# dselivanov/rsparse

Hardware: AMD Instinct MI355X
Metric: als_iterations_per_sec (higher is better)
Workload: dtype f32 (Gram products of rows > 512 / <= 32 non-zeros as 2 x fp16 / 3 x bf16 split terms of the fp32 operands, fp32 accumulate; everything else fp32); 1 GPU; WRMF implicit ALS, CG(3), synthetic 10000000x1000000, 500155883 nnz, rank 128, lambda 0.1; survey_config=3, feedback=implicit, n_items=1000000, nnz=500155883, rank=128, solver=conjugate_gradient, cg_steps=3, parallelism=rows sharded x1, factors replicated

## Files before the change

rsparse_amd/build.py:

```python
import subprocess
import sys
import time
from concurrent.futures import ThreadPoolExecutor
from pathlib import Path

PKG = Path(__file__).resolve().parent
CSRC = PKG / "csrc"
SRC = [CSRC / n for n in ("wrmf_kernels.hip", "wrmf_cgq.hip", "wrmf_cgp.hip", "wrmf_ne.hip", "wrmf_chol.hip", "wrmf_chol_wave.hip", "wrmf_chol_mf.hip", "wrmf_cg_mf.hip", "wrmf_chol_lr.hip",
                          "wrmf_topk.hip", "wrmf_topk_large.hip", "wrmf_similar.hip", "wrmf_metrics.hip", "wrmf_hits.hip", "wrmf_lists.hip", "wrmf_diversity.hip", "wrmf_mmr.hip", "wrmf_ranks.hip", "wrmf_score.hip", "wrmf_softals.hip", "wrmf_itemknn.hip", "wrmf_candidates.hip", "wrmf_sample.hip", "wrmf_sample_weighted.hip", "wrmf_split.hip", "wrmf_confidence.hip", "wrmf_events.hip", "wrmf_explain.hip", "wrmf_init.hip", "wrmf_ingest.hip", "wrmf_nnls.hip", "wrmf_bias.hip", "wrmf_lu.hip",
                          "wrmf_f64.hip", "wrmf_wide.hip", "wrmf_wide_cg.hip", "wrmf_ctx_kernels.hip", "wrmf_schedule.cpp", "wrmf_capi.cpp", "wrmf_f64_capi.cpp", "wrmf_capi_host.cpp", "wrmf_ctx.cpp")]
HEADERS = [CSRC / "wrmf_chol_mf.attrs.csv", CSRC / "wrmf_mf.h", CSRC / "wrmf_internal.h", CSRC / "wrmf_capi_common.h", CSRC / "wrmf_schedule.h", CSRC / "wrmf_device.h", CSRC / "wrmf_sample_team.h", CSRC / "wrmf_wave.h", CSRC / "wrmf_csr_rows.h", CSRC / "wrmf_ldlt.h", CSRC / "wrmf_f64.h", CSRC / "wrmf_topk_plan.h", CSRC / "wrmf_ctx_layout.h", PKG.parent / "include" / "rsparse_wrmf_hip.h"]
DEPS = SRC + HEADERS
OUT = PKG / "lib" / "librsparse_wrmf_hip.so"
FLAGS = ["--offload-arch=gfx950", "-O3", "-std=c++17", "-fPIC"]


EXTRA_FLAGS = {n: ["-mllvm", "-forceattrs-csv-path=" + str(CSRC / "wrmf_chol_mf.attrs.csv"), "-fno-slp-vectorize"] for n in ("wrmf_chol_mf.hip", "wrmf_cg_mf.hip")}
AUDITED = {"wrmf_chol_mf.hip", "wrmf_cg_mf.hip"}
REG_LIMIT = {"wrmf_cg_mf.hip": 512}
NO_SPILL = {"wrmf_cgq.hip": ("14als_cgq_kernelILi128ELi24ELi4ELi4E",),
            "wrmf_cgp.hip": ("14als_cgp_kernelILb0ELb1ELi16ELb1E",),
            "wrmf_explain.hip": ("14explain_kernelIfLi128E",),
            "wrmf_sample.hip": ("13sample_kernelILi64E", "13sample_kernelILi256E"),
            "wrmf_sample_weighted.hip": ("22sample_weighted_kernelILi64E", "22sample_weighted_kernelILi256E"),
            "wrmf_hits.hip": ("18hit_metrics_kernelILb0E", "18hit_metrics_kernelILb1E"),
            "wrmf_lists.hip": ("19list_metrics_kernelILb0E", "19list_metrics_kernelILb1E"),
            "wrmf_diversity.hip": ("21list_diversity_kernelI", "21item_inv_norms_kernelI"),
            "wrmf_mmr.hip": ("10mmr_kernelI",),
            "wrmf_confidence.hip": ("conf_moments_kernel", "conf_moments_finish_kernel", "conf_table_kernel", "conf_apply_kernel"),
            "wrmf_events.hip": ("events_pack_kernel", "events_now_kernel", "events_heads_kernel", "events_reduce_kernel",
                                "events_long_chunks_kernel", "events_long_finish_kernel"),
            "wrmf_cg_mf.hip": ("rsparse_hip_als_cg_mf_implicit", "rsparse_hip_als_cg_mf_implicit_any"),
            "wrmf_softals.hip": ("softals_span_kernel", "softals_finish_kernel", "softals_empty_rows_kernel"),
            "wrmf_itemknn.hip": ("knn_scatter_kernel", "knn_mask_kernel", "knn_select_kernel", "knn_gather_kernel", "knn_cand_select_kernel",
                                 "knn_ranks_kernel"),
            "wrmf_split.hip": ("split_count_wave_kernel", "split_count_team_kernel", "split_write_wave_kernel", "split_write_team_kernel")}
RESOURCE_FLAG = "-Rpass-analysis=kernel-resource-usage"


def resource_violations(remarks, patterns, limit=256):
    import re
    rows, cur = [], None
    for line in remarks.splitlines():
        m = re.search(r"remark:\s+(.*?) \[-Rpass", line)
        if not m:
            continue
        t = m.group(1).strip()
        if t.startswith("Function Name:"):
            cur = {"name": t.split(":", 1)[1].strip()}
            rows.append(cur)
        elif ":" in t and cur is not None:
            k, v = t.rsplit(":", 1)
            cur[k.strip()] = v.strip()
# ... 94 lines not shown
```

rsparse_amd/csrc/wrmf_capi.cpp:

```cpp
#include "../../include/rsparse_wrmf_hip.h"

#include <cxxabi.h>

#include <algorithm>
#include <cfloat>
#include <cmath>
#include <cstdio>
#include <cstdlib>
#include <cstring>
#include <string>
#include <vector>

#include "wrmf_capi_common.h"
#include "wrmf_topk_plan.h"

using namespace rsparse_hip;

struct rsparse_hip_csc {
  DevCSC d;
  int device = 0;
  std::vector<void*> owned;
};

namespace {
// ... 114 lines not shown
  *out = static_cast<const T*>(p);
  return RSPARSE_HIP_OK;
}

int upload_cut(rsparse_hip_csc& m, const NeCut& cut, NeListSet& L) {
  L = NeListSet();
  L.entries = (int)cut.items.size();
  L.nseg = cut.nseg();
  L.nsplit = (int)cut.split_rows.size();
  if (int rc = upload(m, cut.segs, &L.segs)) return rc;
  if (int rc = upload(m, cut.split_rows, &L.split_rows)) return rc;
  return upload(m, cut.split_ptr, &L.split_ptr);
}
int upload_deal(rsparse_hip_csc& m, const NeDeal& deal, NeListSet& L) {
  L.wg = deal.wg();
  if (int rc = upload(m, deal.rows, &L.rows)) return rc;
  return upload(m, deal.ptr, &L.ptr);
}

int build_schedule(rsparse_hip_csc& m, const int32_t* host_col_ptrs) {
  DevCSC& d = m.d;
  int cus = 256;
  HIP_TRY(hipDeviceGetAttribute(&cus, hipDeviceAttributeMultiprocessorCount, m.device));
  d.q_cfg = cgq_default_cfg();
  SchedulePlan plan;
  if (!plan_schedule(host_col_ptrs, d.n_cols, cus, [](int len) { return cgq_bucket_of(len, cgq_default_cfg()); }, plan))
    return fail(RSPARSE_HIP_ERR_INVALID, "col_ptrs is not non-decreasing");
  d.max_len = plan.max_len; d.nnz_long = plan.nnz_long; d.n_empty = plan.n_empty;
  d.short_max = kTileNnz; d.n_long = plan.n_long;
  for (int b = 0; b < 7; b++) d.q_off[b] = plan.off[b];
  for (int b = 0; b < 6; b++) d.q_nnz[b] = plan.nnz[b];
  d.q_pair_first = plan.pair_first; d.q_team4_first = plan.team4_first;
  d.q_team4_wide_first = plan.team4_wide_first;
  d.q_gt32 = plan.gt32; d.q_gt48 = plan.gt48; d.q_lr_first = plan.lr_first; d.q_n_lr = plan.n_lr;
  d.q_n_chol_long = plan.n_chol_long; d.q_n_nec = plan.n_nec;
  int rc;
  if ((rc = upload(m, plan.order, &d.q_order))) return rc;
  if ((rc = upload(m, plan.stream_off, &d.q_stream_off))) return rc;
  if ((rc = upload_cut(m, plan.cut, d.q_ne))) return rc;
  d.q_ne1 = d.q_ne;
  if ((rc = upload_deal(m, plan.fine, d.q_ne))) return rc;
  if ((rc = upload_deal(m, plan.coarse, d.q_ne1))) return rc;
  if (plan.nec_is_ne) {
    d.q_nec = d.q_ne;
  } else {
    if ((rc = upload_cut(m, plan.cut_nec, d.q_nec))) return rc;
    if ((rc = upload_deal(m, plan.nec, d.q_nec))) return rc;
  }
  return RSPARSE_HIP_OK;
}

bool use_cgq(int rank, const void* X, const void* Y) {
  return rank % 4 == 0 && ((reinterpret_cast<uintptr_t>(X) | reinterpret_cast<uintptr_t>(Y)) & 15) == 0;
}

int check_common(int n_rows, int n_cols, const void* col_ptrs, const void* X, const void* Y, int rank) {
  if (n_rows < 0 || n_cols < 0) return fail(RSPARSE_HIP_ERR_INVALID, "negative matrix dimension");
  if (!col_ptrs) return fail(RSPARSE_HIP_ERR_INVALID, "col_ptrs is NULL");
  if (!X || !Y) return fail(RSPARSE_HIP_ERR_INVALID, "X or Y is NULL");
  if (rank <= 0) return fail(RSPARSE_HIP_ERR_INVALID, "rank must be positive");
  if (rank > RSPARSE_HIP_MAX_RANK)
    return fail(RSPARSE_HIP_ERR_UNSUPPORTED, "rank > 256 is not on the device path");
  return RSPARSE_HIP_OK;
}

thread_local int64_t g_fail_carry[2] = {0, 0};
// ... 84 lines not shown
    const int grid = wide_als_grid(d.n_cols);
    const int grid_w = wide_cg_wave_grid(d.n_cols) + wide_cg_team_grid(d.n_cols);
    if ((rc = g_ws.ensure_partials((size_t)grid + (size_t)grid_w))) return rc;
    HIP_TRY(g_ws.wide_m2.ensure(solver == RSPARSE_SOLVER_NNLS ? (size_t)grid * wide_m2_floats_per_wg(rank) : 0));
    HIP_TRY(g_ws.wide_lu.ensure(solver == RSPARSE_SOLVER_CHOLESKY ? (size_t)grid * rank * rank : 0));
    AlsArgs a{};
    a.col_ptrs = d.col_ptrs; a.row_idx = d.row_idx; a.vals = d.vals;
    a.X = d_X; a.Y = d_Y; a.XtX = implicit ? d_XtX : nullptr;
    a.n_cols = d.n_cols; a.k = rank; a.cg_steps = (int)cg_steps;
    a.lambda = (float)lambda; a.lambda_loss = lambda; a.dynamic_lambda = dynamic_lambda ? 1 : 0;
    a.loss_partials = g_ws.partials; a.fail_counter = g_ws.fails;
    a.rhs_vals = bias ? bias->rhs_vals : nullptr;
    a.loss_tgt = bias ? bias->loss_tgt : nullptr;
    a.rhs_init = bias ? bias->rhs_init : nullptr;
    a.loss_tgt_const = bias ? bias->tgt_const : 1.f;
    a.gbias = (solver == RSPARSE_SOLVER_CONJUGATE_GRADIENT && implicit && bias) ? bias->gbias : 0.f;
    const bool wave_cg = wide_cg_wave_supported(a, solver) && (d.q_order || d.max_len <= kWideCgMaxLen);
    hipError_t we = wave_cg ? launch_wide_cg_wave(a, implicit, kWideCgMaxLen, d.max_len > kWideCgMaxLen ? d.q_order : nullptr, 0, s)
                            : launch_als_wide(a, implicit, solver, g_ws.wide_m2, g_ws.wide_lu, s);
    if (we != hipSuccess) return hip_fail(we, wave_cg ? "launch_wide_cg_wave" : "launch_als_wide");
    if ((we = launch_sum_partials(g_ws.partials, wave_cg ? (size_t)grid_w : (size_t)grid, outw, s, g_ws.partials + g_ws.partial_slots())) != hipSuccess)
      return hip_fail(we, "launch_sum_partials");
    return RSPARSE_HIP_OK;
  }
  const bool cg = solver == RSPARSE_SOLVER_CONJUGATE_GRADIENT;
  const bool cgq = cg && use_cgq(rank, d_X, d_Y);
  QSchedule qs;
  qs.order = d.q_order;
  qs.cfg = d.q_cfg;
  qs.pair_first = d.q_pair_first;
  for (int b = 0; b < 7; b++) qs.off[b] = d.q_off[b];
  qs.team4_first = (implicit && bias && bias->gbias != 0.f) ? d.q_off[2] : d.q_team4_first;
  qs.team4_wide_first = (implicit && bias && bias->gbias != 0.f) ? d.q_off[2] : d.q_team4_wide_first;
  qs.pair_wide = cgp_wide_supported(rank, implicit, implicit && bias && bias->gbias != 0.f);
  qs.pair_quad = cgp_quad_supported(rank, implicit, implicit && bias && bias->gbias != 0.f);
  const bool cg_mf = cgq && implicit && !bias && cg_mf_supported(rank, implicit) && d.q_order && d.q_off[1] > d.q_n_nec;
  if (cg_mf) {
    qs.mf_rows = d.q_order + d.q_n_nec;
    qs.mf_n = d.q_off[1] - d.q_n_nec;
  }
  const bool chol_mf = chol_mf_supported(rank) && !cg && solver == RSPARSE_SOLVER_CHOLESKY && !bias && d.q_order && ne_supported(rank) &&
                       use_cgq(rank, d_X, d_Y) && d.q_lr_first > d.q_off[1];
  const int mf_first = d.q_off[1];
  const int n_mf = chol_mf ? d.q_lr_first - mf_first : 0;
  const bool nec_lists = padded_rank(rank) > 64 && d.q_nec.wg > 0 && !chol_mf;
  const bool ne_chol = !cg && solver == RSPARSE_SOLVER_CHOLESKY && !bias && (nec_lists || d.q_ne.wg > 0 || chol_mf) &&
                       ne_supported(rank) && use_cgq(rank, d_X, d_Y);
  qs.ne = (cg_mf || (ne_chol && nec_lists)) ? d.q_nec : ((implicit && padded_rank(rank) == 128) ? d.q_ne : d.q_ne1);
  const size_t chol_base = chol2_loss_slots(d.n_cols);
  const size_t slots = cgq ? cgq_loss_slots(qs, rank, implicit) : (cg ? cg_loss_slots(d.n_cols, d.n_long)
                                   : (solver == RSPARSE_SOLVER_NNLS ? chol_loss_slots(d.n_cols)
                                      : chol_base + (ne_chol ? (size_t)(qs.ne.entries + qs.ne.nsplit) : 0) +
                                            (size_t)(chol_mf ? chol_mf_loss_slots(n_mf, implicit) : 0) + (size_t)kLuGrid));
  if ((rc = g_ws.ensure_partials(slots))) return rc;
  double* out = d_loss_rows_out ? d_loss_rows_out : g_ws.scalars;
  if (d.n_cols == 0) {
    HIP_TRY(hipMemsetAsync(out, 0, sizeof(double), s));
    return RSPARSE_HIP_OK;
  }
  AlsArgs a;
  a.col_ptrs = d.col_ptrs; a.row_idx = d.row_idx; a.vals = d.vals;
  a.X = d_X; a.Y = d_Y; a.XtX = implicit ? d_XtX : nullptr;
  a.long_rows = d.n_long ? d.q_order : nullptr; a.n_long = d.n_long; a.n_cols = d.n_cols;
  a.chol_long_rows = d.q_order; a.n_chol_long = d.q_order ? d.q_n_chol_long : 0;
  a.chol_list = nullptr; a.chol_first = 0; a.chol_n_main = 0; a.chol_empty_first = 0;
  a.lr_rows = nullptr; a.n_lr = 0; a.lr_flags = nullptr; a.lr_M = nullptr; a.lr_n_gt32 = a.lr_n_gt16 = a.lr_n_gt48 = -1; a.lrx = 0;
// ... 1429 lines not shown
```

rsparse_amd/csrc/wrmf_cgq.hip:

```cpp
#include <algorithm>

#include "wrmf_internal.h"
#include "wrmf_device.h"

namespace rsparse_hip {
namespace {

using namespace dev;

constexpr int kGvFirstMinCapq = 16;
constexpr int kStreamPrefixQ = 4;
constexpr int kIdxPrefetchMaxWpr = 2;

constexpr int kMaxSavedSweeps = 4;

template <int KP>
struct QG {
  static constexpr int RPN = KP / 16;
  static constexpr int VW = RPN >= 4 ? 4 : RPN;
  static constexpr int NV = RPN / VW;
  __device__ static __forceinline__ int elem(int i, int r) { return (r / VW) * (16 * VW) + i * VW + (r % VW); }
};

template <int VW>
struct Piece;
template <>
struct Piece<4> { using type = float4; };
template <>
struct Piece<2> { using type = float2; };

__device__ __forceinline__ float groups_reduce_scatter4(const float a0, const float a1, const float a2, const float a3) {
  const auto s01 = __builtin_amdgcn_permlane16_swap(__float_as_uint(a0), __float_as_uint(a1), false, false);
  const float c = __uint_as_float(s01[0]) + __uint_as_float(s01[1]);
  const auto s23 = __builtin_amdgcn_permlane16_swap(__float_as_uint(a2), __float_as_uint(a3), false, false);
  const float d = __uint_as_float(s23[0]) + __uint_as_float(s23[1]);
  const auto t = __builtin_amdgcn_permlane32_swap(__float_as_uint(c), __float_as_uint(d), false, false);
  return __uint_as_float(t[0]) + __uint_as_float(t[1]);
}
template <int KP, int CAPQ, int WAVES, int WPR, int STREAM, bool IMPLICIT, int DMF = 0>
struct QSmem {
  static constexpr size_t gram_floats = (IMPLICIT && DMF != 1) ? (size_t)KP * KP : 0;
  static constexpr size_t vec_floats = IMPLICIT ? (size_t)WAVES * KP : 0;
  static constexpr size_t red_floats = WPR > 1 ? (size_t)2 * WAVES * KP + 2 * WAVES : 0;
  static constexpr bool cv_lds = !STREAM && CAPQ * (KP / 16) > 128;
  static constexpr bool wideq = !STREAM && CAPQ * (KP / 16) > 160;
  static constexpr size_t tsv_floats = (STREAM && !IMPLICIT) ? 0 : (size_t)WAVES * (cv_lds ? 3 : 2) * CAPQ * 4;
  static constexpr size_t pre_floats = STREAM ? (size_t)WAVES * kStreamPrefixQ * 4 * KP : 0;
  static constexpr int dmf_ps = KP + 8, dmf_os = KP + 4;
  static constexpr size_t dmf_floats = DMF ? (size_t)WAVES * dmf_ps + (size_t)WAVES * dmf_os : 0;
  static constexpr size_t pfx_floats =
      (!STREAM && WPR > kIdxPrefetchMaxWpr && (CAPQ == 16 || CAPQ == 20 || CAPQ == 24)) ? (size_t)WAVES * 2 * CAPQ * 4 : 0;
  static constexpr size_t wl_floats = cv_lds ? (size_t)WAVES * 2 : 0;
  static constexpr size_t xs_floats = cv_lds ? (size_t)WAVES * KP : 0;
  static constexpr size_t bytes =
      (gram_floats + vec_floats + red_floats + tsv_floats + pre_floats + dmf_floats + pfx_floats + wl_floats + xs_floats) * 4 + 16;
};

template <int KP, int CAPQ, int WAVES, int WPR, int STREAM, bool IMPLICIT, int DMF = 0, bool GB = false, bool KFULL = false>
__global__ __launch_bounds__(WAVES * 64, 2) void als_cgq_kernel(AlsArgs a, const int32_t* __restrict__ rows, int n_rows,
                                                             int rows_per_team, size_t loss_slot0) {
  using G_ = QG<KP>;
  constexpr int RPN = G_::RPN, VW = G_::VW, NV = G_::NV, CAP = CAPQ * 4, TEAMS = WAVES / WPR;
  using piece_t = typename Piece<VW>::type;
  using SM = QSmem<KP, CAPQ, WAVES, WPR, STREAM, IMPLICIT, DMF>;
  static_assert(WAVES % WPR == 0, "teams must tile the workgroup");
  constexpr bool GRS = RPN == 8 && VW == 4;
  auto groups_all_reduce8 = [](float(&a8)[RPN]) {
    if constexpr (RPN == 8) {
      const float r0 = groups_reduce_scatter4(a8[0], a8[1], a8[2], a8[3]);
      const float r1 = groups_reduce_scatter4(a8[4], a8[5], a8[6], a8[7]);
      float g0[4], g1[4];
      rows_to_all<4>(r0, g0);
      rows_to_all<4>(r1, g1);
#pragma unroll
      for (int e = 0; e < 4; e++) a8[e] = g0[e], a8[4 + e] = g1[e];
    }
  };
  static_assert(!DMF || (IMPLICIT && KP == 128 && WAVES == 4 && WPR == 1 && STREAM == 0), "DMF geometry");
  static_assert(DMF != 1 || CAPQ == 8, "register-resident G terms: only the 8-quad kernel has the 64 registers");
  static_assert(!GB || IMPLICIT, "the global bias of explicit feedback is removed from the data (R/model_WRMF.R:278-282)");
  const float gbias = GB ? a.gbias : 0.f, ltgt = GB ? a.loss_tgt_const : 1.f;
  extern __shared__ __attribute__((aligned(16))) char smem[];
  float* sG = reinterpret_cast<float*>(smem);
  float* sVec = sG + SM::gram_floats;
// ... 103 lines not shown
  float pf_c = 0.f;
  const int team_global = blockIdx.x * TEAMS + team;
  const int total_teams = gridDim.x * TEAMS;

  auto row_index = [&](int itn) { return team_global + itn * total_teams; };
  int row_c = 0, p1_c = 0, p2_c = 0, row_n = 0;
  if (rows_per_team > 0 && row_index(0) < n_rows) {
    row_c = rows[row_index(0)];
    p1_c = a.col_ptrs[row_c];
    p2_c = a.col_ptrs[row_c + 1];
  }
  if (rows_per_team > 1 && row_index(1) < n_rows) row_n = rows[row_index(1)];
  for (int it = 0; it < rows_per_team; ++it) {
    const int ri = row_index(it);
    const bool have = ri < n_rows;
    if (WPR == 1 && !DMF && !have) break;
    const int row = have ? rfl(row_c) : 0;
    const int p1 = have ? rfl(p1_c) : 0;
    const int p2 = have ? rfl(p2_c) : 0;
    constexpr bool META_LATE = WIDEQ && !KFULL;
#define RSP_ADVANCE_META()                                                      \
    {                                                                           \
      int p1_n = 0, p2_n = 0, row_nn = 0;                                       \
      if (it + 1 < rows_per_team && row_index(it + 1) < n_rows) {               \
        p1_n = a.col_ptrs[row_n];                                               \
        p2_n = a.col_ptrs[row_n + 1];                                           \
      }                                                                         \
      if (it + 2 < rows_per_team && row_index(it + 2) < n_rows) row_nn = rows[row_index(it + 2)]; \
      row_c = row_n;                                                            \
      p1_c = p1_n;                                                              \
      p2_c = p2_n;                                                              \
      row_n = row_nn;                                                           \
    }
    if constexpr (!META_LATE) RSP_ADVANCE_META()
    const int cnt = p2 - p1;
    float* yrow = a.Y + (size_t)row * k;
    if (!GB && WPR == 1 && cnt <= 0) {
      if (!DMF || have)
        for (int e = lane; e < k; e += 64) yrow[e] = 0.f;
      if constexpr (!DMF) continue;
    }
    constexpr int PQ = STREAM ? kStreamPrefixQ : 0, PCAP = PQ * 4, PTEAM = PCAP * WPR;
    const int pre = STREAM ? min(cnt, PTEAM) : 0;
    const int pw = STREAM ? max(0, min(PCAP, pre - tw * PCAP)) : 0;
    const int nchunks = (cnt - pre + CAP - 1) / CAP;
    constexpr bool resident = STREAM == 0;
    const float lam_use =
        IMPLICIT ? 0.f : (float)(a.lambda_loss * (a.dynamic_lambda ? (double)(float)cnt : 1.0));

    float* tscr = nullptr;
    float alph[kMaxSavedSweeps];
#pragma unroll
    for (int s2 = 0; s2 < kMaxSavedSweeps; s2++) alph[s2] = 0.f;
    if constexpr (STREAM == 1) {
      if (a.tscr && have && a.cg_steps <= kMaxSavedSweeps) tscr = a.tscr + a.stream_off[ri];
    }

    float xt[CAPQ][RPN];
    float cv[CVLDS ? 1 : CAPQ];
    constexpr int NSL = (CAP + 63) / 64;
    float cl[CVLDS ? 1 : NSL];
#pragma unroll
    for (int s2 = 0; s2 < (CVLDS ? 1 : NSL); s2++) cl[s2] = 0.f;
    auto csv_fill = [&](auto&& conf_of, const int n) {
      const int ln = opaque_lane<WIDEQ>(lane);
#pragma unroll
      for (int s2 = 0; s2 < NSL; s2++) {
        const int sl = ln + 64 * s2;
        if (s2 == 0 || sl < CAP) csv[(sl & 3) * CAPQ + (sl >> 2)] = sl < n ? conf_of(sl) : 0.f;
      }
    };
    int ccnt = 0;
// ... 476 lines not shown
      if (mode != 2) {
#pragma unroll
        for (int rr = 0; rr < RPN; rr++) out[rr] = acc[rr];
        if constexpr (GB) {
          if (mode == 0) {
#pragma unroll
            for (int b = 0; b < NV; b++) {
              const int off = b * 16 * VW + i * VW;
              const piece_t pc = *reinterpret_cast<const piece_t*>(a.rhs_init + min(off, k - VW));
              const float* pf = reinterpret_cast<const float*>(&pc);
#pragma unroll
              for (int c = 0; c < VW; c++) out[b * VW + c] += off < k ? pf[c] : 0.f;
            }
          }
        }
        if constexpr (!IMPLICIT) {
#pragma unroll
          for (int rr = 0; rr < RPN; rr++) out[rr] = fmaf(mode == 0 ? -lam_use : lam_use, v[rr], out[rr]);
        }
      } else {
        loss_out = lacc;
      }
    };

    auto dot16 = [&](const float(&u)[RPN], const float(&w)[RPN]) {
      float s = 0.f;
#pragma unroll
      for (int rr = 0; rr < RPN; rr++) s = fmaf(u[rr], w[rr], s);
      return row16_sum(s);
    };

    const bool live = have && (GB || cnt > 0);
    float dummy = 0.f;
    sweep(x, 0, r, dummy, live);
    auto x_piece = [&](const int b) { return reinterpret_cast<piece_t*>(xs + b * 16 * VW + i * VW); };
    if constexpr (CVLDS) {
      if (g == 0) {
#pragma unroll
        for (int b = 0; b < NV; b++) {
          piece_t pc;
          float* pf = reinterpret_cast<float*>(&pc);
#pragma unroll
          for (int c = 0; c < VW; c++) pf[c] = x[b * VW + c];
          *x_piece(b) = pc;
        }
      }
    }
    if constexpr (META_LATE) RSP_ADVANCE_META()
#undef RSP_ADVANCE_META
    if constexpr (IDXPF && STREAM == 0) {
      if (it + 1 < rows_per_team && row_index(it + 1) < n_rows) {
        const int np1 = rfl(p1_c), ncnt = rfl(p2_c) - np1;
        const int nper = min(CAP, (((ncnt + WPR - 1) / WPR) + 15) & ~15);
        const int ncc = max(0, min(nper, ncnt - tw * nper));
        if (ncc > 0) {
          const int j = np1 + tw * nper + min(lane & (CAP - 1), ncc - 1);
          pf_id = a.row_idx[j];
          pf_c = a.vals[j];
          pf_cnt = ncc;
        }
      }
    }
    if constexpr (DMAPF) {
      if (it + 1 < rows_per_team && row_index(it + 1) < n_rows) {
        const int np1 = rfl(p1_c), ncnt = rfl(p2_c) - np1;
        const int nper = min(CAP, (((ncnt + WPR - 1) / WPR) + 15) & ~15);
        const int ncc = max(0, min(nper, ncnt - tw * nper));
        if (ncc > 0) {
          dma_slot(np1 + tw * nper, ncc);
          pf_cnt = ncc;
        }
      }
    }
#pragma unroll
    for (int rr = 0; rr < RPN; rr++) p[rr] = r[rr];
    float rsold = dot16(r, r);
    bool conv = false;
    for (int itc = 0; itc < a.cg_steps; ++itc) {
      if (WPR == 1 && !DMF && conv) break;
      sweep(p, 1, ap, dummy, live && !conv, itc + 1);
      if (!conv) {
        const float pap = dot16(p, ap);
        const float alpha = (float)((double)rsold / (double)pap);
#pragma unroll
        for (int s2 = 0; s2 < kMaxSavedSweeps; s2++)
          if (s2 == itc) alph[s2] = alpha;
        if constexpr (TSAVE) {
          wave_sync();
          const int ln = opaque_lane<WIDEQ>(lane);
#pragma unroll
          for (int s2 = 0; s2 < NSL; s2++) {
            const int sl = NSL == 1 ? (lane & (CAP - 1)) : ln + 64 * s2;
            if (CAP % 64 == 0 || sl < CAP) tacc[sl] = fmaf(alpha, tcur[sl], tacc[sl]);
          }
          wave_sync();
        }
        if constexpr (CVLDS) {
          if (g == 0) {
#pragma unroll
            for (int b = 0; b < NV; b++) {
              piece_t pc = *x_piece(b);
              float* pf = reinterpret_cast<float*>(&pc);
#pragma unroll
              for (int c = 0; c < VW; c++) pf[c] = fmaf(alpha, p[b * VW + c], pf[c]);
              *x_piece(b) = pc;
// ... 11 lines not shown
        } else {
          const float beta = (float)((double)rsnew / (double)rsold);
#pragma unroll
          for (int rr = 0; rr < RPN; rr++) p[rr] = fmaf(p[rr], beta, r[rr]);
          rsold = rsnew;
        }
      }
    }
    if constexpr (CVLDS) {
      wave_sync();
#pragma unroll
      for (int b = 0; b < NV; b++) {
        const piece_t pc = *x_piece(b);
        const float* pf = reinterpret_cast<const float*>(&pc);
#pragma unroll
        for (int c = 0; c < VW; c++) x[b * VW + c] = pf[c];
      }
    }
    float rl = 0.f;
    sweep(x, 2, ap, rl, live);
    if constexpr (META_LATE) p1_c = rfl(p1_c), p2_c = rfl(p2_c);
    if constexpr (DMAPF) wait_vm<0>();
    if constexpr (IDXPF && STREAM == 0) {
      asm volatile("" : "+v"(pf_id), "+v"(pf_c));
    }
    if (live && tw == 0) {
      const float xx = dot16(x, x);
      const double wl_row = IMPLICIT ? (double)rl + a.lambda_loss * (double)xx : (double)(rl + lam_use * xx);
      if constexpr (CVLDS) {
        if (lane == 0) *wl_lds += wl_row;
      } else {
        wloss += wl_row;
      }
      if (g == 0) {
#pragma unroll
        for (int b = 0; b < NV; b++) {
          const int off = b * 16 * VW + i * VW;
          if (off < k) {
            piece_t pc;
            float* pf = reinterpret_cast<float*>(&pc);
#pragma unroll
            for (int c = 0; c < VW; c++) pf[c] = x[b * VW + c];
            *reinterpret_cast<piece_t*>(yrow + off) = pc;
          }
        }
      }
    }
  }
  if (lane == 0) a.loss_partials[loss_slot0 + (size_t)blockIdx.x * WAVES + wv] = CVLDS ? *wl_lds : wloss;
}

struct BucketDef { int waves, wpr, capq, stream, max_len; };
constexpr int kNB = 6;
constexpr int kNCfg = 2;
constexpr BucketDef kBuckets[kNCfg][kNB] = {
    {{8, 8, 16, 1, 0x7fffffff}, {8, 8, 16, 0, 512}, {4, 4, 16, 0, 256}, {4, 2, 16, 0, 128}, {4, 1, 16, 0, 64}, {4, 1, 8, 0, 32}},
    {{8, 8, 16, 1, 0x7fffffff}, {4, 4, 32, 0, 512}, {4, 2, 32, 0, 256}, {4, 1, 32, 0, 128}, {4, 1, 16, 0, 64}, {4, 1, 8, 0, 32}},
};
constexpr int cfg_of_kp(int KP) { return KP == 64 ? 1 : 0; }
constexpr int kTeam4Waves = 4, kTeam4Capq = 20;
static_assert(kTeam4Max == kTeam4Waves * kTeam4Capq * 4, "wrmf_internal.h's split and the kernel's capacity");
constexpr int kTeam4WideCapq = 24;
static_assert(kTeam4WideMax == kTeam4Waves * kTeam4WideCapq * 4, "wrmf_schedule.h's split and the wide kernel's capacity");
static_assert(kTeam4Max < kTeam4WideMax && kTeam4WideMax < 512, "the 4-wave launches take bucket 1's rows from its short end");
static_assert(QSmem<128, kTeam4WideCapq, kTeam4Waves, kTeam4Waves, 0, true>::bytes <= 80 * 1024, "the wide team kernel's LDS");
constexpr bool team4_split(int KP, bool GB) { return KP == 128 && !GB; }
int team4_first(const QSchedule& q) { return std::min(std::max(q.team4_first, q.off[1]), q.off[2]); }
int team4_wide_first(const QSchedule& q) { return std::min(std::max(q.team4_wide_first, q.off[1]), team4_first(q)); }

template <int KP, int WAVES, int CAPQ, int WPR, int STREAM, bool IMPLICIT, bool GB, int DMF = 0, bool KFULL = false>
hipError_t launch_bucket(const AlsArgs& a, const int32_t* rows, int n_rows, int grid, size_t slot0, hipStream_t s,
                         hipEvent_t* ev_slot) {
  if (n_rows <= 0) return hipSuccess;
  constexpr bool kDmfGeometry = IMPLICIT && KP == 128 && WAVES == 4 && WPR == 1 && (CAPQ == 8 || CAPQ == 16) && STREAM == 0;
  if constexpr (kDmfGeometry && !DMF) {
    return launch_bucket<KP, WAVES, CAPQ, WPR, STREAM, IMPLICIT, GB, CAPQ == 8 ? 1 : 2>(a, rows, n_rows, grid, slot0, s, ev_slot);
  } else {
    if constexpr (!KFULL && STREAM == 0 && !(DMF == 1 && !GB)) {
      if (a.k == KP)
        return launch_bucket<KP, WAVES, CAPQ, WPR, STREAM, IMPLICIT, GB, DMF, true>(a, rows, n_rows, grid, slot0, s, ev_slot);
    }
    constexpr int TEAMS = WAVES / WPR;
    auto kern = als_cgq_kernel<KP, CAPQ, WAVES, WPR, STREAM, IMPLICIT, DMF, GB, KFULL>;
    const size_t lds = QSmem<KP, CAPQ, WAVES, WPR, STREAM, IMPLICIT, DMF>::bytes;
    hipError_t err = hipFuncSetAttribute(reinterpret_cast<const void*>(kern),
                                         hipFuncAttributeMaxDynamicSharedMemorySize, (int)lds);
    if (err != hipSuccess) return err;
    const int total_teams = grid * TEAMS;
    const int rpt = (n_rows + total_teams - 1) / total_teams;
    prof_note(ev_slot, reinterpret_cast<const void*>(kern));
    hipLaunchKernelGGL(kern, dim3(grid), dim3(WAVES * 64), lds, s, a, rows, n_rows, rpt, slot0);
    return hipGetLastError();
  }
}

struct BucketStreams {
  hipStream_t st[kNB] = {nullptr, nullptr, nullptr, nullptr, nullptr, nullptr};
  hipEvent_t fork = nullptr, fork0 = nullptr;
  hipEvent_t done[kNB] = {nullptr, nullptr, nullptr, nullptr, nullptr, nullptr};
  int device = -1;
  hipError_t ensure() {
    int dev = 0;
    hipError_t err = hipGetDevice(&dev);
    if (err != hipSuccess) return err;
    if (dev == device) return hipSuccess;
    device = dev;
    if ((err = hipEventCreateWithFlags(&fork, hipEventDisableTiming)) != hipSuccess) return err;
    if ((err = hipEventCreateWithFlags(&fork0, hipEventDisableTiming)) != hipSuccess) return err;
    for (int b = 0; b < kNB; b++) {
      if ((err = hipStreamCreateWithFlags(&st[b], hipStreamNonBlocking)) != hipSuccess) return err;
      if ((err = hipEventCreateWithFlags(&done[b], hipEventDisableTiming)) != hipSuccess) return err;
    }
    return hipSuccess;
  }
};
thread_local BucketStreams g_bs;

int g_launch_mode = 2;
int concurrent_buckets() { return g_launch_mode; }

size_t bucket_slots(const QSchedule& q, int b, int k, bool implicit) {
  const int cfg = cfg_of_kp(padded_rank(k));
  const BucketDef d = kBuckets[cfg][b];
  if (d.wpr <= 0) return 0;
  if (d.stream && ne_supported(k)) return (size_t)(q.ne.entries + q.ne.nsplit) + (size_t)(q.mf_n > 0 ? cg_mf_loss_slots(q.mf_n) : 0);
  const int rows = q.off[b + 1] - q.off[b];
  if (b == 1 && padded_rank(k) == 128) {
    const int wide = team4_wide_first(q), split = team4_first(q);
    return (size_t)cgq_bucket_grid(wide - q.off[b], b, cfg) * d.waves + (size_t)cgq_team4_wide_grid(split - wide) * kTeam4Waves +
           (size_t)cgq_team4_grid(q.off[b + 1] - split) * kTeam4Waves;
  }
  if (b == kNB - 1 && rows > 0 && cgp_supported(k, implicit)) {
    const int split = std::min(std::max(q.pair_first, q.off[b]), q.off[b + 1]);
    const size_t main = q.pair_wide ? (size_t)cgp_loss_slots(split - q.off[b], cgp_rows_per_wave(kCgpWide))
                                    : (size_t)cgq_bucket_grid(split - q.off[b], b, cfg) * d.waves;
    return main + (size_t)cgp_loss_slots(q.off[b + 1] - split, cgp_rows_per_wave(q.pair_quad ? kCgpQuad : kCgpPair));
  }
  return (size_t)cgq_bucket_grid(rows, b, cfg) * d.waves;
}

template <int KP, int CFG, bool IMPLICIT, bool GB>
hipError_t launch_all(const AlsArgs& a, const QSchedule& q, hipStream_t s, hipEvent_t* ev) {
  hipError_t err;
  size_t slot = 0;
  const int cmode = ev ? 0 : concurrent_buckets();
  const bool overlap = cmode != 0;
  bool forked = false;
  if (overlap) {
    if ((err = g_bs.ensure()) != hipSuccess) return err;
  }
#define RSP_BUCKET(B)                                                                                       \
  {                                                                                                         \
    constexpr BucketDef D = kBuckets[CFG][B];                                                               \
    if (ev && (err = hipEventRecord(ev[B], s)) != hipSuccess) return err;                                   \
    if constexpr (D.wpr > 0) {                                                                              \
      const int n = q.off[B + 1] - q.off[B];                                                                \
      const int grid = cgq_bucket_grid(n, B, CFG);                                                          \
      if (n > 0) {                                                                                          \
        hipStream_t bs = s;                                                                                 \
        const bool side = overlap && !(cmode == 2 && D.stream);                                             \
        if (side) {                                                                                         \
          if (!forked) {                                                                                    \
            if ((err = hipEventRecord(g_bs.fork, s)) != hipSuccess) return err;                             \
// ... 17 lines not shown
            hipStream_t ms = bs;                                                                            \
            if (mside) {                                                                                    \
              ms = g_bs.st[B];                                                                              \
              if ((err = hipStreamWaitEvent(ms, g_bs.fork0, 0)) != hipSuccess) return err;                  \
            }                                                                                               \
            if ((err = launch_als_cg_mf(a, q.mf_rows, q.mf_n, (int)(slot + (size_t)(q.ne.entries + q.ne.nsplit)), ms, \
                                        ev ? ev + B : nullptr)) != hipSuccess)                              \
              return err;                                                                                   \
            if (mside) {                                                                                    \
              if ((err = hipEventRecord(g_bs.done[B], ms)) != hipSuccess) return err;                       \
              if ((err = hipStreamWaitEvent(s, g_bs.done[B], 0)) != hipSuccess) return err;                 \
            }                                                                                               \
          }                                                                                                 \
        } else if constexpr (D.stream && KP > 32) {        \
          return hipErrorInvalidValue;                                                                      \
        } else if constexpr (B == 1 && team4_split(KP, GB)) {                                              \
           \
           \
          const int first = q.off[B], wide = team4_wide_first(q), split = team4_first(q);                   \
          const int n_main = wide - first, n_w4 = split - wide, n_t4 = q.off[B + 1] - split;                \
          const int g_main = cgq_bucket_grid(n_main, B, CFG), g_w4 = cgq_team4_wide_grid(n_w4);             \
          if ((err = launch_bucket<KP, D.waves, D.capq, D.wpr, D.stream, IMPLICIT, GB>(a, q.order + first, n_main, g_main, slot, \
                                                                                  bs, ev ? ev + B : nullptr)) != hipSuccess) \
            return err;                                                                                     \
          if ((err = launch_bucket<KP, kTeam4Waves, kTeam4WideCapq, kTeam4Waves, 0, IMPLICIT, GB>(          \
                   a, q.order + wide, n_w4, g_w4, slot + (size_t)g_main * D.waves, bs,                      \
                   n_main > 0 ? nullptr : (ev ? ev + B : nullptr))) != hipSuccess)                          \
            return err;                                                                                     \
          if ((err = launch_bucket<KP, kTeam4Waves, kTeam4Capq, kTeam4Waves, 0, IMPLICIT, GB>(              \
                   a, q.order + split, n_t4, cgq_team4_grid(n_t4),                                          \
                   slot + (size_t)g_main * D.waves + (size_t)g_w4 * kTeam4Waves, bs,                        \
                   n_main + n_w4 > 0 ? nullptr : (ev ? ev + B : nullptr))) != hipSuccess)                   \
            return err;                                                                                     \
        } else if (B == kNB - 1 && cgp_supported(a.k, IMPLICIT)) {                    \
           \
                  \
          const int first = q.off[B], split = std::min(std::max(q.pair_first, first), q.off[B + 1]);         \
          const int n_main = split - first, n_pair = q.off[B + 1] - split;                                   \
          size_t main_slots;                                                                                \
          if (q.pair_wide) {                                                                                \
            if ((err = launch_als_cgp(a, q.order + first, n_main, kCgpWide, slot, bs, ev ? ev + B : nullptr)) != hipSuccess) \
              return err;                                                                                   \
            main_slots = (size_t)cgp_loss_slots(n_main, cgp_rows_per_wave(kCgpWide));                       \
          } else {                                                                                          \
            const int g_main = cgq_bucket_grid(n_main, B, CFG);                                             \
            if ((err = launch_bucket<KP, D.waves, D.capq, D.wpr, D.stream, IMPLICIT, GB>(a, q.order + first, n_main, g_main, slot, \
                                                                                    bs, ev ? ev + B : nullptr)) != hipSuccess) \
              return err;                                                                                   \
            main_slots = (size_t)g_main * D.waves;                                                          \
          }                                                                                                 \
          if ((err = launch_als_cgp(a, q.order + split, n_pair, q.pair_quad ? kCgpQuad : kCgpPair, slot + main_slots, bs, \
                                    n_main > 0 ? nullptr : (ev ? ev + B : nullptr))) != hipSuccess)           \
            return err;                                                                                     \
        } else if ((err = launch_bucket<KP, D.waves, D.capq, D.wpr, D.stream, IMPLICIT, GB>(a, q.order + q.off[B], n, grid, slot, \
                                                                                bs, ev ? ev + B : nullptr)) != hipSuccess) \
          return err;                                                                                       \
        if (side) {                                                                                         \
          if ((err = hipEventRecord(g_bs.done[B], bs)) != hipSuccess) return err;                           \
          if ((err = hipStreamWaitEvent(s, g_bs.done[B], 0)) != hipSuccess) return err;                     \
        }                                                                                                   \
      }                                                                                                     \
      slot += bucket_slots(q, B, a.k, IMPLICIT);                                                             \
    }                                                                                                       \
  }
  RSP_BUCKET(0)
  RSP_BUCKET(1)
// ... 73 lines not shown
```

rsparse_amd/csrc/wrmf_internal.h:

```cpp
#pragma once
#include <hip/hip_runtime.h>
#include <cstdint>
#include <string>

#include "wrmf_schedule.h"

namespace rsparse_hip {

constexpr float kCgTol = 1e-10f;
constexpr double kCgTolD = 1e-10;
constexpr int kScdMaxIter = 10000;
constexpr float kScdTol = 1e-4f;
constexpr double kScdTolD = 1e-4;
constexpr float kNnlsEps = 1e-16f;
constexpr double kNnlsEpsD = 1e-16;

struct NeListSet {
  const int32_t* rows = nullptr;
  const int32_t* ptr = nullptr;
  int wg = 0;
  int entries = 0;
  const int32_t* segs = nullptr;
  int nseg = 0;
  const int32_t* split_rows = nullptr;
  const int32_t* split_ptr = nullptr;
  int nsplit = 0;
};

struct DevCSC {
  int n_rows = 0;
  int n_cols = 0;
  int64_t nnz = 0;
  const int32_t* col_ptrs = nullptr;
  const int32_t* row_idx = nullptr;
  const float* vals = nullptr;
  int n_long = 0;
  int short_max = 0;
  int max_len = 0;
  const int32_t* q_order = nullptr;
  int q_off[7] = {0, 0, 0, 0, 0, 0, 0};
  int q_cfg = 0;
  int q_pair_first = 0;
  int q_team4_first = 0;
  int q_team4_wide_first = 0;
  int64_t q_nnz[6] = {0, 0, 0, 0, 0, 0};
  const int64_t* q_stream_off = nullptr;
  int q_n_chol_long = 0;
  int q_gt32 = 0;
  int q_gt48 = 0;
  int q_lr_first = 0, q_n_lr = 0;
  NeListSet q_ne;
  NeListSet q_ne1;
  int q_n_nec = 0;
  NeListSet q_nec;
  int64_t nnz_long = 0;
  int n_empty = 0;
  mutable bool vals_frozen = false;
  mutable bool vstats_valid = false;
  mutable unsigned* vstats = nullptr;
  mutable hipStream_t vstats_stream = nullptr;
};

struct AlsArgs {
  const int32_t* col_ptrs;
  const int32_t* row_idx;
  const float* vals;
  const float* X;
  float* Y;
  const float* XtX;
  const int32_t* long_rows;
  int n_long;
  int n_cols;
  int k;
  int cg_steps;
  float lambda;
  double lambda_loss;
  int dynamic_lambda;
// ... 11 lines not shown
  const int32_t* ne_r0_slot;
  float* tscr;
  const int64_t* stream_off;
  int64_t stream_nnz;
  const int32_t* chol_long_rows;
  int n_chol_long;
  const int32_t* chol_list;
  int chol_first, chol_n_main, chol_empty_first;
  const int32_t* lr_rows;
  int n_lr;
  int lr_n_gt32, lr_n_gt16;
  int lr_n_gt48;
  float* nnls_lhs;
  const int32_t* nnls_order;
  int lrx;
  unsigned* lr_flags;
  float* lr_M;
  const int32_t* ne_segs;
  float* ne_seg_scratch;
  int* ne_seg_flags;
  int ne_chol;
  int ne_chol_min;
  const unsigned* ne_stats;
  const float* mf_XtX;
  const unsigned* wave_stats;
};

struct QSchedule {
  const int32_t* order;
  int off[7];
  int pair_first;
  int team4_first;
  int team4_wide_first;
  bool pair_wide;
  bool pair_quad = false;
  int cfg;
  NeListSet ne;
  const int32_t* mf_rows = nullptr;
  int mf_n = 0;
};
int cgq_default_cfg();
void cgq_set_launch_mode(int mode);
int cgq_num_buckets();
int cgq_bucket_wpr(int cfg, int b);
int cgq_bucket_capq(int cfg, int b);
int cgq_bucket_waves(int cfg, int b);
int cgq_bucket_stream(int cfg, int b);
int cgq_bucket_grid(int n_rows, int bucket, int cfg);
int cgq_team4_grid(int n_rows);
int cgq_team4_wide_grid(int n_rows);
int cgq_bucket_of(int len, int cfg);
size_t cgq_loss_slots(const QSchedule& q, int k, bool implicit);
bool cgp_supported(int k, bool implicit);
bool cgp_wide_supported(int k, bool implicit, bool gbias);
bool cgp_quad_supported(int k, bool implicit, bool gbias);
enum CgpForm { kCgpPair = 0, kCgpWide = 1, kCgpQuad = 2 };
inline int cgp_rows_per_wave(CgpForm form) { return form == kCgpQuad ? 4 : 2; }
hipError_t launch_als_cgp(const AlsArgs& a, const int32_t* rows, int n_rows, CgpForm form, size_t loss_slot0, hipStream_t s,
                          hipEvent_t* ev_slot);
bool ne_supported(int k);
constexpr int kNeMinLen = 512;
constexpr int kNeSegFloats = 4 * (11 * 16 * 64 + 128 + 2);
hipError_t launch_ne_stats(const float* X, int64_t nx, const float* vals, int64_t nnz, unsigned* stats, hipStream_t s,
                           const float* absmax_hint = nullptr, const unsigned* cached_vstats = nullptr,
                           unsigned* save_vstats = nullptr);
hipError_t launch_als_ne(const AlsArgs& a, const QSchedule& q, bool implicit, double* row_loss, hipStream_t s,
// ... 311 lines not shown
```

rsparse_amd/csrc/wrmf_schedule.cpp:

```cpp
#include "wrmf_schedule.h"

#include <algorithm>
#include <functional>
#include <queue>
#include <utility>

namespace rsparse_hip {

namespace {
int ne_slots(int cus) { return 2 * std::max(cus, 1); }
}

int cgp_grid(int n_rows, int rows_per_wave) {
  if (n_rows <= 0) return 0;
  const long sets = ((long)n_rows + rows_per_wave - 1) / rows_per_wave;
  long per_wave = 32;
  const long spread = 4L * 512;
  if (sets < spread * per_wave) per_wave = (sets + spread - 1) / spread;
  if (per_wave < 1) per_wave = 1;
  return (int)((sets + 4 * per_wave - 1) / (4 * per_wave));
}
int cgp_visits(int n_rows, int rows_per_wave) {
  const long grid = cgp_grid(n_rows, rows_per_wave);
  if (grid <= 0) return 0;
  const long sets = ((long)n_rows + rows_per_wave - 1) / rows_per_wave;
  return (int)((sets + grid * 4 - 1) / (grid * 4));
}
int64_t cgp_loss_slots(int n_rows, int rows_per_wave) { return (int64_t)cgp_grid(n_rows, rows_per_wave) * 4; }

NeCut ne_cut(const int32_t* order, const int32_t* col_ptrs, int n_prefix, int64_t fixed, int cus) {
  NeCut c;
  if (n_prefix <= 0) return c;
  auto len_of = [&](int r) { return (int64_t)(col_ptrs[order[r] + 1] - col_ptrs[order[r]]); };
  auto steps_of = [](int64_t len) { return (len + 15) / 16; };
  const int n_slots = ne_slots(cus);
  int64_t total = 0;
  for (int r = 0; r < n_prefix; r++) total += steps_of(len_of(r)) + fixed;
  const int64_t share = std::max<int64_t>(1, total / n_slots);
  c.items.reserve((size_t)n_prefix + 64);
  int n_seg = 0;
  for (int r = 0; r < n_prefix; r++) {
    const int64_t len = len_of(r);
    const int64_t st = steps_of(len);
    int parts = 1;
    if (n_slots >= 8 && 2 * (st + fixed) > share)
      parts = (int)std::min<int64_t>(std::min<int64_t>(kNeMaxSeg, st / 64), (4 * st + share - 1) / share);
    if (parts < 2 || n_seg + parts > kNeMaxSegTotal) {
      c.items.push_back({st + fixed, order[r]});
      continue;
    }
    const int64_t per = (st + parts - 1) / parts;
    const int slot = n_seg;
    const int made = (int)((st + per - 1) / per);
    int idx = 0;
    for (int64_t s0 = 0; s0 < st; s0 += per, idx++) {
      const int64_t n0 = s0 * 16, n1 = std::min(len, (s0 + per) * 16);
      c.segs.insert(c.segs.end(), {order[r], (int32_t)n0, (int32_t)(n1 - n0), idx, made, slot});
      c.items.push_back({steps_of(n1 - n0) + fixed, -(int32_t)(n_seg + 1)});
      n_seg++;
    }
    c.split_rows.push_back(-(int32_t)(slot + 1));
// ... 26 lines not shown
  d.rows.resize(n_items);
  std::vector<int32_t> fill(d.ptr.begin(), d.ptr.end() - 1);
  for (size_t e = 0; e < n_items; e++) d.rows[(size_t)fill[(size_t)owner[e]]++] = cut.items[e].entry;
  return d;
}

bool plan_schedule(const int32_t* col_ptrs, int n_cols, int cus, int (*bucket_of)(int len), SchedulePlan& out) {
  out = SchedulePlan();
  const int n = n_cols;
  int max_len = 0;
  for (int i = 0; i < n; i++) {
    const int len = col_ptrs[i + 1] - col_ptrs[i];
    if (len < 0) return false;
    max_len = std::max(max_len, len);
  }
  out.max_len = max_len;
  if (n <= 0) {
    out.nec_is_ne = true;
    return true;
  }
  std::vector<int64_t> start((size_t)max_len + 2, 0);
  for (int i = 0; i < n; i++) start[(size_t)(max_len - (col_ptrs[i + 1] - col_ptrs[i])) + 1]++;
  int cnt_b[6] = {0, 0, 0, 0, 0, 0};
  for (int len = max_len; len >= 0; len--) {
    const int cnt = (int)start[(size_t)(max_len - len) + 1];
    if (!cnt) continue;
    if (len > kTileNnz) { out.n_long += cnt; out.nnz_long += (int64_t)len * cnt; }
    if (len == 0) out.n_empty += cnt;
    if (len > kCholLongLen) out.n_chol_long += cnt;
    if (len > kCgMfMax) out.n_nec += cnt;
    if (len > 16) out.pair_first += cnt;
    if (len > kTeam4Max) out.team4_first += cnt;
    if (len > kTeam4WideMax) out.team4_wide_first += cnt;
    if (len > 32) out.gt32 += cnt;
    if (len > 48) out.gt48 += cnt;
    if (len > kCholLrMax) out.lr_first += cnt;
    else if (len >= 1) out.n_lr += cnt;
    const int b = bucket_of(len);
    cnt_b[b] += cnt;
    out.nnz[b] += (int64_t)len * cnt;
  }
  for (int b = 0; b < 6; b++) out.off[b + 1] = out.off[b] + cnt_b[b];
  for (size_t b = 1; b < start.size(); b++) start[b] += start[b - 1];
  out.order.resize((size_t)n);
  for (int i = 0; i < n; i++) out.order[(size_t)start[(size_t)(max_len - (col_ptrs[i + 1] - col_ptrs[i]))]++] = i;
  const int n_stream = out.off[1];
  if (n_stream > 0) {
    out.stream_off.assign((size_t)n_stream + 1, 0);
    for (int r = 0; r < n_stream; r++) {
      const int row = out.order[(size_t)r];
      out.stream_off[(size_t)r + 1] = out.stream_off[(size_t)r] + (col_ptrs[row + 1] - col_ptrs[row]);
    }
    out.cut = ne_cut(out.order.data(), col_ptrs, n_stream, 12, cus);
    out.fine = ne_deal(out.cut, n_stream, cus, true);
    out.coarse = ne_deal(out.cut, n_stream, cus, false);
  }
  out.nec_is_ne = out.n_nec == n_stream;
  if (!out.nec_is_ne) {
    out.cut_nec = ne_cut(out.order.data(), col_ptrs, out.n_nec, 12, cus);
    out.nec = ne_deal(out.cut_nec, out.n_nec, cus, true);
  }
  return true;
}

}
```

rsparse_amd/csrc/wrmf_schedule.h:

```cpp
#pragma once
#include <cstdint>
#include <vector>

namespace rsparse_hip {

constexpr int kTileNnz = 32;
constexpr int kTeam4Max = 320;
constexpr int kTeam4WideMax = 384;
constexpr int kCholLrMax = 64;
constexpr int kCholLongLen = 4096;
constexpr int kCgMfMax = 16384;
constexpr int kNeMaxSeg = 16;
constexpr int kNeMaxSegTotal = 1024;

int cgp_grid(int n_rows, int rows_per_wave = 2);
int cgp_visits(int n_rows, int rows_per_wave = 2);
int64_t cgp_loss_slots(int n_rows, int rows_per_wave = 2);

struct NeCut {
  struct Item { int64_t cost; int32_t entry; };
  std::vector<Item> items;
  std::vector<int32_t> segs;
  std::vector<int32_t> split_rows;
  std::vector<int32_t> split_ptr;
  int nseg() const { return (int)(segs.size() / 6); }
};
struct NeDeal {
  std::vector<int32_t> rows, ptr;
  int wg() const { return ptr.empty() ? 0 : (int)ptr.size() - 1; }
};

NeCut ne_cut(const int32_t* order, const int32_t* col_ptrs, int n_prefix, int64_t fixed, int cus);
NeDeal ne_deal(const NeCut& cut, int n_prefix, int cus, bool fine);

struct SchedulePlan {
  int max_len = 0;
  int n_long = 0;
  int64_t nnz_long = 0;
  int n_empty = 0;
  std::vector<int32_t> order;
  int off[7] = {0, 0, 0, 0, 0, 0, 0};
  int64_t nnz[6] = {0, 0, 0, 0, 0, 0};
  int pair_first = 0;
  int team4_first = 0;
  int team4_wide_first = 0;
  int gt32 = 0, gt48 = 0;
  int lr_first = 0, n_lr = 0;
  int n_chol_long = 0;
  int n_nec = 0;
  std::vector<int64_t> stream_off;
  NeCut cut, cut_nec;
  NeDeal fine, coarse, nec;
  bool nec_is_ne = false;
};

bool plan_schedule(const int32_t* col_ptrs, int n_cols, int cus, int (*bucket_of)(int len), SchedulePlan& out);

}
```

Measured before the change: 8.657 iterations/s.

## Split bucket 3's short rows into a one-wave wide-queue CG kernel launch

Adds a schedule split point so bucket 3 rows with at most 96 non-zeros go to a dedicated launch: one wave per row, 4 waves per workgroup, queue capacity 24, with its own grid and loss-slot sizing. The kernel gains a wide-queue one-wave path that moves the metadata advance to the middle of the row, makes index values wave-uniform via readfirstlane and opaque lane tricks, and enables LDS index prefetch for CAPQ above 16. The goal is better occupancy and latency hiding for mid-length rows than the generic bucket configuration gives. It adds another launch, more template instantiations and register pressure, and the no-spill guard pattern is loosened so it covers the new instantiation.

```diff
diff --git a/rsparse_amd/build.py b/rsparse_amd/build.py
--- a/rsparse_amd/build.py
+++ b/rsparse_amd/build.py
@@ -18,7 +18,8 @@
 EXTRA_FLAGS = {n: ["-mllvm", "-forceattrs-csv-path=" + str(CSRC / "wrmf_chol_mf.attrs.csv"), "-fno-slp-vectorize"] for n in ("wrmf_chol_mf.hip", "wrmf_cg_mf.hip")}
 AUDITED = {"wrmf_chol_mf.hip", "wrmf_cg_mf.hip"}
 REG_LIMIT = {"wrmf_cg_mf.hip": 512}
-NO_SPILL = {"wrmf_cgq.hip": ("14als_cgq_kernelILi128ELi24ELi4ELi4E",),
+NO_SPILL = {
+            "wrmf_cgq.hip": ("14als_cgq_kernelILi128ELi24ELi4ELi",),
             "wrmf_cgp.hip": ("14als_cgp_kernelILb0ELb1ELi16ELb1E",),
             "wrmf_explain.hip": ("14explain_kernelIfLi128E",),
             "wrmf_sample.hip": ("13sample_kernelILi64E", "13sample_kernelILi256E"),
diff --git a/rsparse_amd/csrc/wrmf_capi.cpp b/rsparse_amd/csrc/wrmf_capi.cpp
--- a/rsparse_amd/csrc/wrmf_capi.cpp
+++ b/rsparse_amd/csrc/wrmf_capi.cpp
@@ -170,6 +170,7 @@
   for (int b = 0; b < 6; b++) d.q_nnz[b] = plan.nnz[b];
   d.q_pair_first = plan.pair_first; d.q_team4_first = plan.team4_first;
   d.q_team4_wide_first = plan.team4_wide_first;
+  d.q_wave1_wide_first = plan.wave1_wide_first;
   d.q_gt32 = plan.gt32; d.q_gt48 = plan.gt48; d.q_lr_first = plan.lr_first; d.q_n_lr = plan.n_lr;
   d.q_n_chol_long = plan.n_chol_long; d.q_n_nec = plan.n_nec;
   int rc;
@@ -320,6 +321,7 @@
   for (int b = 0; b < 7; b++) qs.off[b] = d.q_off[b];
   qs.team4_first = (implicit && bias && bias->gbias != 0.f) ? d.q_off[2] : d.q_team4_first;
   qs.team4_wide_first = (implicit && bias && bias->gbias != 0.f) ? d.q_off[2] : d.q_team4_wide_first;
+  qs.wave1_wide_first = (implicit && bias && bias->gbias != 0.f) ? d.q_off[4] : d.q_wave1_wide_first;
   qs.pair_wide = cgp_wide_supported(rank, implicit, implicit && bias && bias->gbias != 0.f);
   qs.pair_quad = cgp_quad_supported(rank, implicit, implicit && bias && bias->gbias != 0.f);
   const bool cg_mf = cgq && implicit && !bias && cg_mf_supported(rank, implicit) && d.q_order && d.q_off[1] > d.q_n_nec;
diff --git a/rsparse_amd/csrc/wrmf_cgq.hip b/rsparse_amd/csrc/wrmf_cgq.hip
--- a/rsparse_amd/csrc/wrmf_cgq.hip
+++ b/rsparse_amd/csrc/wrmf_cgq.hip
@@ -49,7 +49,7 @@
   static constexpr int dmf_ps = KP + 8, dmf_os = KP + 4;
   static constexpr size_t dmf_floats = DMF ? (size_t)WAVES * dmf_ps + (size_t)WAVES * dmf_os : 0;
   static constexpr size_t pfx_floats =
-      (!STREAM && WPR > kIdxPrefetchMaxWpr && (CAPQ == 16 || CAPQ == 20 || CAPQ == 24)) ? (size_t)WAVES * 2 * CAPQ * 4 : 0;
+      (!STREAM && (WPR > kIdxPrefetchMaxWpr || CAPQ > 16) && (CAPQ == 16 || CAPQ == 20 || CAPQ == 24)) ? (size_t)WAVES * 2 * CAPQ * 4 : 0;
   static constexpr size_t wl_floats = cv_lds ? (size_t)WAVES * 2 : 0;
   static constexpr size_t xs_floats = cv_lds ? (size_t)WAVES * KP : 0;
   static constexpr size_t bytes =
@@ -219,12 +219,14 @@
       p2_c = p2_n;                                                              \
       row_n = row_nn;                                                           \
     }
-    if constexpr (!META_LATE) RSP_ADVANCE_META()
+    constexpr bool META_MID = WIDEQ && WPR == 1 && KFULL;
+    if constexpr (!META_LATE && !META_MID) RSP_ADVANCE_META()
     const int cnt = p2 - p1;
     float* yrow = a.Y + (size_t)row * k;
     if (!GB && WPR == 1 && cnt <= 0) {
       if (!DMF || have)
-        for (int e = lane; e < k; e += 64) yrow[e] = 0.f;
+        for (int e = opaque_lane<SM::wideq && WPR == 1>(lane); e < k; e += 64) yrow[e] = 0.f;
+      if constexpr (META_MID) RSP_ADVANCE_META()
       if constexpr (!DMF) continue;
     }
     constexpr int PQ = STREAM ? kStreamPrefixQ : 0, PCAP = PQ * 4, PTEAM = PCAP * WPR;
@@ -767,8 +769,12 @@
 
     const bool live = have && (GB || cnt > 0);
     float dummy = 0.f;
+    if constexpr (META_MID) RSP_ADVANCE_META()
     sweep(x, 0, r, dummy, live);
-    auto x_piece = [&](const int b) { return reinterpret_cast<piece_t*>(xs + b * 16 * VW + i * VW); };
+    auto x_piece = [&](const int b) {
+      const int is = (WIDEQ && WPR == 1) ? (opaque_lane<WIDEQ && WPR == 1>(lane) & 15) : i;
+      return reinterpret_cast<piece_t*>(xs + b * 16 * VW + is * VW);
+    };
     if constexpr (CVLDS) {
       if (g == 0) {
 #pragma unroll
@@ -803,9 +809,10 @@
         const int ncc = max(0, min(nper, ncnt - tw * nper));
         if (ncc > 0) {
           dma_slot(np1 + tw * nper, ncc);
-          pf_cnt = ncc;
-        }
-      }
+          pf_cnt = (WIDEQ && WPR == 1) ? rfl(ncc) : ncc;
+        }
+      }
+      if constexpr (WIDEQ && WPR == 1 && !META_LATE) p1_c = rfl(p1_c), p2_c = rfl(p2_c);
     }
 #pragma unroll
     for (int rr = 0; rr < RPN; rr++) p[rr] = r[rr];
@@ -883,10 +890,11 @@
       } else {
         wloss += wl_row;
       }
+      const int is = (WIDEQ && WPR == 1) ? (opaque_lane<WIDEQ && WPR == 1>(lane) & 15) : i;
       if (g == 0) {
 #pragma unroll
         for (int b = 0; b < NV; b++) {
-          const int off = b * 16 * VW + i * VW;
+          const int off = b * 16 * VW + is * VW;
           if (off < k) {
             piece_t pc;
             float* pf = reinterpret_cast<float*>(&pc);
@@ -916,8 +924,15 @@
 static_assert(kTeam4Max < kTeam4WideMax && kTeam4WideMax < 512, "the 4-wave launches take bucket 1's rows from its short end");
 static_assert(QSmem<128, kTeam4WideCapq, kTeam4Waves, kTeam4Waves, 0, true>::bytes <= 80 * 1024, "the wide team kernel's LDS");
 constexpr bool team4_split(int KP, bool GB) { return KP == 128 && !GB; }
+constexpr int kWave1WideWaves = 4, kWave1WideCapq = 24;
+static_assert(kWave1WideMax == kWave1WideCapq * 4, "wrmf_schedule.h's split and the one-wave wide kernel's capacity");
+static_assert(kWave1WideMax > kBuckets[0][4].max_len && kWave1WideMax < kBuckets[0][3].max_len,
+              "the one-wave launch takes bucket 3's rows from its short end");
+static_assert(QSmem<128, kWave1WideCapq, kWave1WideWaves, 1, 0, true>::bytes <= 80 * 1024, "the one-wave wide kernel's LDS");
+constexpr bool wave1_split(int KP, bool IMPLICIT, bool GB) { return KP == 128 && IMPLICIT && !GB; }
 int team4_first(const QSchedule& q) { return std::min(std::max(q.team4_first, q.off[1]), q.off[2]); }
 int team4_wide_first(const QSchedule& q) { return std::min(std::max(q.team4_wide_first, q.off[1]), team4_first(q)); }
+int wave1_wide_first(const QSchedule& q) { return std::min(std::max(q.wave1_wide_first, q.off[3]), q.off[4]); }
 
 template <int KP, int WAVES, int CAPQ, int WPR, int STREAM, bool IMPLICIT, bool GB, int DMF = 0, bool KFULL = false>
 hipError_t launch_bucket(const AlsArgs& a, const int32_t* rows, int n_rows, int grid, size_t slot0, hipStream_t s,
@@ -980,6 +995,10 @@
     const int wide = team4_wide_first(q), split = team4_first(q);
     return (size_t)cgq_bucket_grid(wide - q.off[b], b, cfg) * d.waves + (size_t)cgq_team4_wide_grid(split - wide) * kTeam4Waves +
            (size_t)cgq_team4_grid(q.off[b + 1] - split) * kTeam4Waves;
+  }
+  if (b == 3 && k == 128 && implicit) {
+    const int split = wave1_wide_first(q);
+    return (size_t)cgq_bucket_grid(split - q.off[b], b, cfg) * d.waves + (size_t)cgq_wave1_wide_loss_slots(q.off[b + 1] - split);
   }
   if (b == kNB - 1 && rows > 0 && cgp_supported(k, implicit)) {
     const int split = std::min(std::max(q.pair_first, q.off[b]), q.off[b + 1]);
@@ -1063,6 +1082,21 @@
                    slot + (size_t)g_main * D.waves + (size_t)g_w4 * kTeam4Waves, bs,                        \
                    n_main + n_w4 > 0 ? nullptr : (ev ? ev + B : nullptr))) != hipSuccess)                   \
             return err;                                                                                     \
+        } else if (B == 3 && wave1_split(KP, IMPLICIT, GB) && a.k == KP) {                                  \
+           \
+                         \
+          if constexpr (B == 3 && wave1_split(KP, IMPLICIT, GB)) {                                          \
+            const int first = q.off[B], split = wave1_wide_first(q);                                        \
+            const int n_main = split - first, n_w1 = q.off[B + 1] - split;                                  \
+            const int g_main = cgq_bucket_grid(n_main, B, CFG);                                             \
+            if ((err = launch_bucket<KP, D.waves, D.capq, D.wpr, D.stream, IMPLICIT, GB>(a, q.order + first, n_main, g_main, slot, \
+                                                                                    bs, ev ? ev + B : nullptr)) != hipSuccess) \
+              return err;                                                                                   \
+            if ((err = launch_bucket<KP, kWave1WideWaves, kWave1WideCapq, 1, 0, IMPLICIT, GB, 0, true>(     \
+                     a, q.order + split, n_w1, cgq_wave1_wide_grid(n_w1), slot + (size_t)g_main * D.waves, bs, \
+                     n_main > 0 ? nullptr : (ev ? ev + B : nullptr))) != hipSuccess)                        \
+              return err;                                                                                   \
+          }                                                                                                 \
         } else if (B == kNB - 1 && cgp_supported(a.k, IMPLICIT)) {                    \
            \
                   \
diff --git a/rsparse_amd/csrc/wrmf_internal.h b/rsparse_amd/csrc/wrmf_internal.h
--- a/rsparse_amd/csrc/wrmf_internal.h
+++ b/rsparse_amd/csrc/wrmf_internal.h
@@ -43,6 +43,7 @@
   int q_pair_first = 0;
   int q_team4_first = 0;
   int q_team4_wide_first = 0;
+  int q_wave1_wide_first = 0;
   int64_t q_nnz[6] = {0, 0, 0, 0, 0, 0};
   const int64_t* q_stream_off = nullptr;
   int q_n_chol_long = 0;
@@ -120,6 +121,7 @@
   int pair_first;
   int team4_first;
   int team4_wide_first;
+  int wave1_wide_first;
   bool pair_wide;
   bool pair_quad = false;
   int cfg;
diff --git a/rsparse_amd/csrc/wrmf_schedule.cpp b/rsparse_amd/csrc/wrmf_schedule.cpp
--- a/rsparse_amd/csrc/wrmf_schedule.cpp
+++ b/rsparse_amd/csrc/wrmf_schedule.cpp
@@ -27,6 +27,20 @@
   return (int)((sets + grid * 4 - 1) / (grid * 4));
 }
 int64_t cgp_loss_slots(int n_rows, int rows_per_wave) { return (int64_t)cgp_grid(n_rows, rows_per_wave) * 4; }
+
+int cgq_wave1_wide_grid(int n_rows) {
+  if (n_rows <= 0) return 0;
+  long per_wave = 64;
+  const long spread = 4L * 512;
+  if ((long)n_rows < spread * per_wave) per_wave = ((long)n_rows + spread - 1) / spread;
+  if (per_wave < 1) per_wave = 1;
+  return (int)(((long)n_rows + 4 * per_wave - 1) / (4 * per_wave));
+}
+int cgq_wave1_wide_visits(int n_rows) {
+  const long waves = 4L * cgq_wave1_wide_grid(n_rows);
+  return waves <= 0 ? 0 : (int)(((long)n_rows + waves - 1) / waves);
+}
+int64_t cgq_wave1_wide_loss_slots(int n_rows) { return (int64_t)cgq_wave1_wide_grid(n_rows) * 4; }
 
 NeCut ne_cut(const int32_t* order, const int32_t* col_ptrs, int n_prefix, int64_t fixed, int cus) {
   NeCut c;
@@ -119,6 +133,7 @@
     if (len > 16) out.pair_first += cnt;
     if (len > kTeam4Max) out.team4_first += cnt;
     if (len > kTeam4WideMax) out.team4_wide_first += cnt;
+    if (len > kWave1WideMax) out.wave1_wide_first += cnt;
     if (len > 32) out.gt32 += cnt;
     if (len > 48) out.gt48 += cnt;
     if (len > kCholLrMax) out.lr_first += cnt;
diff --git a/rsparse_amd/csrc/wrmf_schedule.h b/rsparse_amd/csrc/wrmf_schedule.h
--- a/rsparse_amd/csrc/wrmf_schedule.h
+++ b/rsparse_amd/csrc/wrmf_schedule.h
@@ -7,6 +7,7 @@
 constexpr int kTileNnz = 32;
 constexpr int kTeam4Max = 320;
 constexpr int kTeam4WideMax = 384;
+constexpr int kWave1WideMax = 96;
 constexpr int kCholLrMax = 64;
 constexpr int kCholLongLen = 4096;
 constexpr int kCgMfMax = 16384;
@@ -16,6 +17,10 @@
 int cgp_grid(int n_rows, int rows_per_wave = 2);
 int cgp_visits(int n_rows, int rows_per_wave = 2);
 int64_t cgp_loss_slots(int n_rows, int rows_per_wave = 2);
+
+int cgq_wave1_wide_grid(int n_rows);
+int cgq_wave1_wide_visits(int n_rows);
+int64_t cgq_wave1_wide_loss_slots(int n_rows);
 
 struct NeCut {
   struct Item { int64_t cost; int32_t entry; };
@@ -44,6 +49,7 @@
   int pair_first = 0;
   int team4_first = 0;
   int team4_wide_first = 0;
+  int wave1_wide_first = 0;
   int gt32 = 0, gt48 = 0;
   int lr_first = 0, n_lr = 0;
   int n_chol_long = 0;
```

New measurement: 8.700 iterations/s (median of 6 runs). About the same (+0.5%).
